# fingltd/4mc

Hardware: AMD Instinct MI355X
Metric: GB/s compress+decompress (silesia-like S-mix, 4mc-Fast) (higher is better)
Workload: dtype u8; 1 GPU; 4mc Fast (LZ4 fast), 4 MiB blocks, corpus replicated to 8.00 GiB per GPU, HBM resident; blocks_per_gpu=2048, block_bytes=4194304, parallelism=block-range dp1, arch=gfx950:sramecc+:xnack-

## Files before the change

4mc_amd/csrc/lz4_emit.hip:

```cpp
#include <hip/hip_runtime.h>
#include <stdint.h>
#include "fourmc_gpu.h"
#include "kernels.h"
#include "lz4emit.h"

namespace {

constexpr uint32_t kEmitGroups = 8;
constexpr int      kEmitThreads = 256;

__global__ __launch_bounds__(kEmitThreads)
void lz4_emit_kernel(const uint8_t* __restrict__ src_base, uint8_t* __restrict__ dst_base, const fourmc_block* blocks,
                     uint32_t nblocks, const uint8_t* __restrict__ work, uint32_t reccap)
{
    const uint32_t b = blockIdx.x / kEmitGroups, g = blockIdx.x % kEmitGroups;
    if (b >= nblocks) return;
    const uint32_t cnt = reinterpret_cast<const uint32_t*>(work)[b];
    if (cnt == 0) return;
    const fourmc_block blk = uniform_block(blocks[b]);
    const uint8_t* src = src_base + blk.src_off;
    uint8_t* dst = dst_base + blk.dst_off;
    if (cnt == kRecRawCopy) {
        const uint32_t n = blk.src_len;
        const uint32_t slice = ((n + kEmitGroups - 1) / kEmitGroups + 15) & ~15u;
        const uint32_t lo = min(n, g * slice), hi = min(n, lo + slice);
        copy_group<kEmitThreads>(dst + lo, src + lo, hi - lo, int(threadIdx.x));
        return;
    }
    const uint4* rec = reinterpret_cast<const uint4*>(work + lz4rec_count_bytes(nblocks) + size_t(b) * lz4rec_area_bytes(reccap));
    const uint32_t wave = threadIdx.x / 64;
    const int lane = int(threadIdx.x % 64);
    constexpr uint32_t kWaves = kEmitThreads / 64;
    for (uint32_t t = g * kWaves + wave; size_t(t) * 64 < cnt; t += kEmitGroups * kWaves)
        emit_records(rec, t * 64, cnt, 0, src, dst, lane);
}

}

extern "C" hipError_t fourmc_launch_lz4_emit(const void* d_src, void* d_dst, const fourmc_block* d_blocks, uint32_t n,
                                             const void* d_work, uint32_t reccap, hipStream_t stream)
{
    if (n == 0) return hipSuccess;
    hipLaunchKernelGGL(lz4_emit_kernel, dim3(n * kEmitGroups), dim3(kEmitThreads), 0, stream,
                       static_cast<const uint8_t*>(d_src), static_cast<uint8_t*>(d_dst), d_blocks, n,
                       static_cast<const uint8_t*>(d_work), reccap);
    return hipGetLastError();
}
```

4mc_amd/csrc/pack.hip:

```cpp
#include <hip/hip_runtime.h>
#include <stdint.h>
#include "fourmc_gpu.h"
#include "kernels.h"

namespace {

struct __attribute__((packed, aligned(1))) U16B { uint32_t x, y, z, w; };

__global__ __launch_bounds__(256)
void pack_image_kernel(const uint8_t* __restrict__ staging, uint8_t* __restrict__ image,
                       const fourmc_block* __restrict__ blocks, const uint64_t* __restrict__ image_off,
                       uint32_t nblocks)
{
    const uint32_t b = blockIdx.x;
    if (b >= nblocks) return;
    const fourmc_block blk = blocks[b];
    const uint32_t csize = blk.result > 0 ? uint32_t(blk.result) : 0u;
    uint8_t* out = image + image_off[b];
    const uint8_t* in = staging + blk.dst_off;
    const uint32_t t = threadIdx.x;
    if (t < 12) {
        const uint32_t field = t < 4 ? blk.src_len : (t < 8 ? csize : blk.xxh32);
        out[t] = uint8_t(field >> (8 * (3 - (t & 3))));
    }
    out += 12;
    const uint32_t head = min(csize, uint32_t((16 - (reinterpret_cast<uintptr_t>(out) & 15)) & 15));
    if (t < head) out[t] = in[t];
    const uint32_t body = (csize - head) & ~15u;
    for (uint32_t k = 16 * t; k < body; k += 16 * 256) {
        const U16B v = *reinterpret_cast<const U16B*>(in + head + k);
        *reinterpret_cast<uint4*>(out + head + k) = make_uint4(v.x, v.y, v.z, v.w);
    }
    const uint32_t tail0 = head + body;
    if (tail0 + t < csize) out[tail0 + t] = in[tail0 + t];
}

}

extern "C" hipError_t fourmc_launch_pack_image(const void* d_staging, void* d_image, const fourmc_block* d_blocks,
                                               const uint64_t* d_image_off, uint32_t n, hipStream_t stream)
{
    if (n == 0) return hipSuccess;
    hipLaunchKernelGGL(pack_image_kernel, dim3(n), dim3(256), 0, stream,
                       static_cast<const uint8_t*>(d_staging), static_cast<uint8_t*>(d_image), d_blocks, d_image_off, n);
    return hipGetLastError();
}
```

Baseline: 36.80 GB/s.

## Stage short LZ4 sequences in LDS and split image packing across groups

The LZ4 emit kernel now gives each wavefront a contiguous range of record batches. It prefetches the next records and their literals, and writes short sequences (token, up to 32 literal bytes, offset, short length) into a per-wave LDS buffer, which is then flushed to global memory with aligned 16-byte stores. Long literals are copied cooperatively by the whole wave, and other records take a per-lane path. The pack kernel now splits each block's copy across 8 workgroups in 256 KiB slices instead of one workgroup per block. The aim is fewer scattered byte stores and more parallel bandwidth, at the cost of a more complex emit path, LDS pressure and extra ballot loops.

```diff
diff --git a/4mc_amd/csrc/lz4_emit.hip b/4mc_amd/csrc/lz4_emit.hip
--- a/4mc_amd/csrc/lz4_emit.hip
+++ b/4mc_amd/csrc/lz4_emit.hip
@@ -8,11 +8,169 @@
 
 constexpr uint32_t kEmitGroups = 8;
 constexpr int      kEmitThreads = 256;
+constexpr uint32_t kEmitWaves = kEmitGroups * (kEmitThreads / 64);
+constexpr uint32_t kLaneLit = 64;
+constexpr uint32_t kStageLit = 32;
+constexpr uint32_t kStageLen = 4;
+constexpr uint32_t kStageRec = 1 + 1 + kStageLit + 2 + kStageLen;
+constexpr uint32_t kStage = 64 * kStageRec + 16;
+static_assert(kStage % 16 == 0 && 8 * (kEmitThreads / 64) * kStage <= 160 * 1024, "32 wavefronts a CU");
+
+__device__ __forceinline__ uint4 load_record(const uint4* rec, uint32_t i, uint32_t cnt) { return rec[min(i, cnt - 1)]; }
+
+__device__ __forceinline__ void arrive(U16B& v) { asm volatile("" : "+v"(v.a), "+v"(v.b)); }
+__device__ __forceinline__ void arrive(uint4& v) { asm volatile("" : "+v"(v.x), "+v"(v.y), "+v"(v.z), "+v"(v.w)); }
+
+__device__ __forceinline__ uint32_t len_bytes(uint32_t v) { return v >= 15 ? (v - 15) / 255 + 1 : 0; }
+
+__device__ __forceinline__ void flush_range(const uint8_t* st, uint32_t ls, uint8_t* g, uint32_t k, int lane)
+{
+    const uint32_t head = min(k, (16u - (ls & 15u)) & 15u);
+    if (uint32_t(lane) < head) g[lane] = st[ls + lane];
+    const uint32_t body = (k - head) & ~15u;
+    for (uint32_t j = 16u * uint32_t(lane); j < body; j += 16 * 64)
+        *reinterpret_cast<uint4*>(g + head + j) = *reinterpret_cast<const uint4*>(st + ls + head + j);
+    const uint32_t t0 = head + body;
+    if (t0 + uint32_t(lane) < k) g[t0 + lane] = st[ls + t0 + lane];
+}
+
+__device__ __forceinline__ void copy_wave(uint8_t* d, const uint8_t* s, uint32_t k, int lane)
+{
+    constexpr uint32_t S = 16 * 64;
+    for (; k; ) {
+        const uint32_t c = min(k, 4 * S), j = 16u * uint32_t(lane);
+        const bool h0 = j + 16 <= c, h1 = j + S + 16 <= c, h2 = j + 2 * S + 16 <= c, h3 = j + 3 * S + 16 <= c;
+        const uint32_t tj = c & ~15u, tr = c & 15u;
+        const bool mine = tr != 0 && ((tj >> 4) & 63u) == uint32_t(lane);
+        const uint32_t o8 = tj, o4 = o8 + (tr & 8), o2 = o4 + (tr & 4), o1 = o2 + (tr & 2);
+        U16B p0 = {0, 0}, p1 = {0, 0}, p2 = {0, 0}, p3 = {0, 0};
+        uint64_t t8 = 0; uint32_t t4 = 0, t2 = 0, t1 = 0;
+        if (h0) p0 = ld16u(s + j);
+        if (h1) p1 = ld16u(s + j + S);
+        if (h2) p2 = ld16u(s + j + 2 * S);
+        if (h3) p3 = ld16u(s + j + 3 * S);
+        if (mine && (tr & 8)) t8 = ld8(s + o8);
+        if (mine && (tr & 4)) t4 = ld4(s + o4);
+        if (mine && (tr & 2)) t2 = ld2u(s + o2);
+        if (mine && (tr & 1)) t1 = s[o1];
+        arrive(p0); arrive(p1); arrive(p2); arrive(p3);
+        asm volatile("" : "+v"(t8), "+v"(t4), "+v"(t2), "+v"(t1));
+        if (h0) st16u(d + j, p0);
+        if (h1) st16u(d + j + S, p1);
+        if (h2) st16u(d + j + 2 * S, p2);
+        if (h3) st16u(d + j + 3 * S, p3);
+        if (mine && (tr & 8)) st8u(d + o8, t8);
+        if (mine && (tr & 4)) st4u(d + o4, t4);
+        if (mine && (tr & 2)) st2u(d + o2, uint16_t(t2));
+        if (mine && (tr & 1)) d[o1] = uint8_t(t1);
+        d += c; s += c; k -= c;
+    }
+}
+
+__device__ __forceinline__ void copy_lane_once(uint8_t* d, const uint8_t* s, uint32_t k)
+{
+    if (k >= 32) {
+        U16B a = ld16u(s), b = ld16u(s + 16), c = ld16u(s + k - 32), e = ld16u(s + k - 16);
+        arrive(a); arrive(b); arrive(c); arrive(e);
+        st16u(d, a); st16u(d + 16, b); st16u(d + k - 32, c); st16u(d + k - 16, e);
+    } else if (k >= 16) {
+        U16B a = ld16u(s), e = ld16u(s + k - 16);
+        arrive(a); arrive(e);
+        st16u(d, a); st16u(d + k - 16, e);
+    } else if (k >= 8) {
+        const uint64_t a = ld8(s), e = ld8(s + k - 8);
+        st8u(d, a); st8u(d + k - 8, e);
+    } else if (k >= 4) {
+        const uint32_t a = ld4(s), e = ld4(s + k - 4);
+        st4u(d, a); st4u(d + k - 4, e);
+    } else if (k >= 2) {
+        const uint16_t a = ld2u(s), e = ld2u(s + k - 2);
+        st2u(d, a); st2u(d + k - 2, e);
+    } else if (k) d[0] = s[0];
+}
+
+__device__ __forceinline__ bool quick_record(uint4 r, bool act, uint32_t n) { return act && r.z <= kStageLit && r.y <= n - kStageLit; }
+
+__device__ __forceinline__ void emit_batch(uint4 r, uint32_t first, bool act, U16B l0, U16B l1, const uint8_t* src, uint32_t n,
+                                           uint8_t* dst, uint8_t* st, int lane)
+{
+    const uint32_t lit = r.z;
+    const bool quick = quick_record(r, act, n);
+    const uint32_t up = uint32_t(__shfl_down(int(r.y), 1));
+    const bool last = (r.w & kRecLast) != 0;
+    const uint32_t mcode = last ? 0u : (lane == 63 ? first : up) - r.y - lit - 4;
+    const uint32_t mext = len_bytes(mcode);
+    const uint32_t len = 1 + len_bytes(lit) + lit + (last ? 0u : 2u + mext);
+    const uint32_t tok = (min(lit, 15u) << 4) | min(mcode, 15u);
+
+    bool staged = quick && mext <= kStageLen;
+    const uint32_t x0 = uint32_t(__builtin_amdgcn_readfirstlane(int(r.x)));
+    uint32_t ls = uint32_t(reinterpret_cast<uintptr_t>(dst + x0) & 15) + (r.x - x0);
+    for (unsigned long long m = __ballot(act && !staged); m; m &= m - 1) {
+        const int d = __builtin_ctzll(m);
+        const uint32_t cut = uint32_t(__builtin_amdgcn_readlane(int(len), d)) & ~15u;
+        if (lane > d) ls -= cut;
+    }
+    staged = staged && ls + len <= kStage;
+
+    if (staged) {
+        st[ls] = uint8_t(tok);
+        if (lit >= 15) st[ls + 1] = uint8_t(lit - 15);
+    }
+    const uint32_t lq = ls + 1 + len_bytes(lit), slit = staged ? lit : 0u;
+    const uint64_t w[4] = {l0.a, l0.b, l1.a, l1.b};
+#pragma unroll
+    for (uint32_t i = 0; i < kStageLit; ++i) {
+        if (i % 8 == 0 && __ballot(i < slit) == 0) break;
+        if (i < slit) st[lq + i] = uint8_t(w[i >> 3] >> (8 * (i & 7)));
+    }
+    if (staged && !last) {
+        const uint32_t q = lq + lit;
+        st[q] = uint8_t(r.w); st[q + 1] = uint8_t(r.w >> 8);
+        if (mcode >= 15) {
+            const uint32_t rest = mcode - 15, n255 = rest / 255;
+#pragma unroll
+            for (uint32_t j = 0; j < kStageLen - 1; ++j) if (j < n255) st[q + 2 + j] = 255;
+            st[q + 2 + n255] = uint8_t(rest - n255 * 255);
+        }
+    }
+
+    uint32_t p = r.x;
+    bool longlit = false;
+    if (act && !staged) {
+        dst[p++] = uint8_t(tok);
+        if (lit >= 15) p += put_len(dst + p, lit - 15);
+        longlit = lit > kLaneLit;
+        if (!longlit) copy_lane_once(dst + p, src + r.y, lit);
+        if (!last) {
+            const uint32_t q = p + lit;
+            st2u(dst + q, uint16_t(r.w));
+            if (mcode >= 15) put_len(dst + q + 2, mcode - 15);
+        }
+    }
+    for (unsigned long long lng = __ballot(longlit); lng; lng &= lng - 1) {
+        const int l = __builtin_ctzll(lng);
+        const uint32_t lp = uint32_t(__builtin_amdgcn_readlane(int(p), l)), lsrc = uint32_t(__builtin_amdgcn_readlane(int(r.y), l));
+        copy_wave(dst + lp, src + lsrc, uint32_t(__builtin_amdgcn_readlane(int(lit), l)), lane);
+    }
+
+    const uint32_t end = ls + len;
+    for (unsigned long long m = __ballot(staged); m; ) {
+        const int a = __builtin_ctzll(m);
+        const unsigned long long rest = ~(m >> a);
+        const int run = rest ? __builtin_ctzll(rest) : 64;
+        const int b = a + run - 1;
+        const uint32_t from = uint32_t(__builtin_amdgcn_readlane(int(ls), a)), to = uint32_t(__builtin_amdgcn_readlane(int(end), b));
+        flush_range(st, from, dst + uint32_t(__builtin_amdgcn_readlane(int(r.x), a)), to > from ? to - from : 0u, lane);
+        m = b >= 63 ? 0ull : m & (~0ull << (b + 1));
+    }
+}
 
 __global__ __launch_bounds__(kEmitThreads)
 void lz4_emit_kernel(const uint8_t* __restrict__ src_base, uint8_t* __restrict__ dst_base, const fourmc_block* blocks,
                      uint32_t nblocks, const uint8_t* __restrict__ work, uint32_t reccap)
 {
+    __shared__ __attribute__((aligned(16))) uint8_t stage[kEmitThreads / 64][kStage];
     const uint32_t b = blockIdx.x / kEmitGroups, g = blockIdx.x % kEmitGroups;
     if (b >= nblocks) return;
     const uint32_t cnt = reinterpret_cast<const uint32_t*>(work)[b];
@@ -20,19 +178,35 @@
     const fourmc_block blk = uniform_block(blocks[b]);
     const uint8_t* src = src_base + blk.src_off;
     uint8_t* dst = dst_base + blk.dst_off;
+    const uint32_t n = blk.src_len;
     if (cnt == kRecRawCopy) {
-        const uint32_t n = blk.src_len;
         const uint32_t slice = ((n + kEmitGroups - 1) / kEmitGroups + 15) & ~15u;
         const uint32_t lo = min(n, g * slice), hi = min(n, lo + slice);
         copy_group<kEmitThreads>(dst + lo, src + lo, hi - lo, int(threadIdx.x));
         return;
     }
     const uint4* rec = reinterpret_cast<const uint4*>(work + lz4rec_count_bytes(nblocks) + size_t(b) * lz4rec_area_bytes(reccap));
-    const uint32_t wave = threadIdx.x / 64;
     const int lane = int(threadIdx.x % 64);
-    constexpr uint32_t kWaves = kEmitThreads / 64;
-    for (uint32_t t = g * kWaves + wave; size_t(t) * 64 < cnt; t += kEmitGroups * kWaves)
-        emit_records(rec, t * 64, cnt, 0, src, dst, lane);
+    const uint32_t w = g * (kEmitThreads / 64) + threadIdx.x / 64;
+    const uint32_t nbatch = (cnt + 63) / 64, per = (nbatch + kEmitWaves - 1) / kEmitWaves;
+    const uint32_t t0 = min(nbatch, w * per), t1 = min(nbatch, t0 + per);
+    if (n < 64) {
+        for (uint32_t t = t0; t < t1; ++t) emit_records(rec, t * 64, cnt, 0, src, dst, lane);
+        return;
+    }
+    if (t0 == t1) return;
+    uint8_t* st = stage[threadIdx.x / 64];
+    uint4 r = load_record(rec, t0 * 64 + uint32_t(lane), cnt), rn = load_record(rec, (t0 + 1) * 64 + uint32_t(lane), cnt);
+    const uint8_t* s0 = src + (quick_record(r, t0 * 64 + uint32_t(lane) < cnt, n) ? r.y : 0u);
+    U16B l0 = ld16u(s0), l1 = ld16u(s0 + 16);
+    for (uint32_t t = t0; t < t1; ++t) {
+        arrive(rn); arrive(l0); arrive(l1);
+        uint4 rnn = load_record(rec, (t + 2) * 64 + uint32_t(lane), cnt);
+        const uint8_t* sn = src + (quick_record(rn, (t + 1) * 64 + uint32_t(lane) < cnt, n) ? rn.y : 0u);
+        const U16B n0 = ld16u(sn), n1 = ld16u(sn + 16);
+        emit_batch(r, uint32_t(__builtin_amdgcn_readfirstlane(int(rn.y))), t * 64 + uint32_t(lane) < cnt, l0, l1, src, n, dst, st, lane);
+        r = rn; rn = rnn; l0 = n0; l1 = n1;
+    }
 }
 
 }
diff --git a/4mc_amd/csrc/pack.hip b/4mc_amd/csrc/pack.hip
--- a/4mc_amd/csrc/pack.hip
+++ b/4mc_amd/csrc/pack.hip
@@ -2,37 +2,38 @@
 #include <stdint.h>
 #include "fourmc_gpu.h"
 #include "kernels.h"
+#include "lz4emit.h"
 
 namespace {
 
-struct __attribute__((packed, aligned(1))) U16B { uint32_t x, y, z, w; };
+constexpr uint32_t kPackGroups  = 8;
+constexpr int      kPackThreads = 256;
+constexpr uint32_t kPackSlice   = 256u << 10;
 
-__global__ __launch_bounds__(256)
+__global__ __launch_bounds__(kPackThreads)
 void pack_image_kernel(const uint8_t* __restrict__ staging, uint8_t* __restrict__ image,
                        const fourmc_block* __restrict__ blocks, const uint64_t* __restrict__ image_off,
                        uint32_t nblocks)
 {
-    const uint32_t b = blockIdx.x;
+    const uint32_t b = blockIdx.x / kPackGroups, g = blockIdx.x % kPackGroups;
     if (b >= nblocks) return;
     const fourmc_block blk = blocks[b];
     const uint32_t csize = blk.result > 0 ? uint32_t(blk.result) : 0u;
     uint8_t* out = image + image_off[b];
     const uint8_t* in = staging + blk.dst_off;
     const uint32_t t = threadIdx.x;
-    if (t < 12) {
+    if (g == 0 && t < 12) {
         const uint32_t field = t < 4 ? blk.src_len : (t < 8 ? csize : blk.xxh32);
         out[t] = uint8_t(field >> (8 * (3 - (t & 3))));
     }
     out += 12;
-    const uint32_t head = min(csize, uint32_t((16 - (reinterpret_cast<uintptr_t>(out) & 15)) & 15));
-    if (t < head) out[t] = in[t];
-    const uint32_t body = (csize - head) & ~15u;
-    for (uint32_t k = 16 * t; k < body; k += 16 * 256) {
-        const U16B v = *reinterpret_cast<const U16B*>(in + head + k);
-        *reinterpret_cast<uint4*>(out + head + k) = make_uint4(v.x, v.y, v.z, v.w);
+    const uint32_t mis = uint32_t((16 - (reinterpret_cast<uintptr_t>(out) & 15)) & 15);
+    for (uint32_t lo = g * kPackSlice; lo < csize; lo += kPackGroups * kPackSlice) {
+        const uint32_t n = min(kPackSlice, csize - lo);
+        const uint32_t head = min(n, mis);
+        if (t < head) out[lo + t] = in[lo + t];
+        copy_group<kPackThreads>(out + lo + head, in + lo + head, n - head, int(t));
     }
-    const uint32_t tail0 = head + body;
-    if (tail0 + t < csize) out[tail0 + t] = in[tail0 + t];
 }
 
 }
@@ -41,7 +42,7 @@
                                                const uint64_t* d_image_off, uint32_t n, hipStream_t stream)
 {
     if (n == 0) return hipSuccess;
-    hipLaunchKernelGGL(pack_image_kernel, dim3(n), dim3(256), 0, stream,
+    hipLaunchKernelGGL(pack_image_kernel, dim3(n * kPackGroups), dim3(kPackThreads), 0, stream,
                        static_cast<const uint8_t*>(d_staging), static_cast<uint8_t*>(d_image), d_blocks, d_image_off, n);
     return hipGetLastError();
 }
```

After: 37.00 GB/s (median of 6 runs). About the same (+0.5%).
